# rhofield/rho-tts

Hardware: AMD Instinct MI355X
Metric: audio-sec/wall-sec (RTF) Qwen3-TTS-1.7B batch=32 (higher is better)
Workload: dtype bf16; 1 GPU; Qwen3-TTS-1.7B bf16, batch 32/GPU, 30-s reference clone, 10-word sentences (44 frames each), sampling=top-k 50 T 0.9, seeded synthetic weights; value counts delivered (post-processed) audio; global_batch=32, parallelism=dp1

## Files before the change

### rho_tts_amd/csrc/common.h

```cpp
#pragma once

#include <hip/hip_runtime.h>

#include <cstdarg>
#include <cstdio>
#include <cstring>
#include <atomic>
#include <mutex>
#include <shared_mutex>
#include <string>
#include <vector>

#include "../../include/rho_tts_amd_debug.h"

struct rt_ctx {
    int device = 0;
    hipStream_t own_stream = nullptr;
    hipStream_t stream = nullptr;
    std::mutex mu;
    std::string last_error;
    int n_cu = 0;
    char arch[64] = {0};
    void* d_scratch = nullptr;
    size_t d_scratch_bytes = 0;
// ... 86 lines not shown
    float o;
    o = dpp_lane_f32<0xB1>(v);  v = o > v ? o : v;
    o = dpp_lane_f32<0x4E>(v);  v = o > v ? o : v;
    o = dpp_lane_f32<0x141>(v); v = o > v ? o : v;
    o = dpp_lane_f32<0x140>(v); v = o > v ? o : v;
    const int x = __float_as_int(v);
    const float r0 = __int_as_float(__builtin_amdgcn_readlane(x, 0)), r1 = __int_as_float(__builtin_amdgcn_readlane(x, 16));
    const float r2 = __int_as_float(__builtin_amdgcn_readlane(x, 32)), r3 = __int_as_float(__builtin_amdgcn_readlane(x, 48));
    const float a = r1 > r0 ? r1 : r0, b = r3 > r2 ? r3 : r2;
    return b > a ? b : a;
}
__device__ __forceinline__ unsigned wave_scan_incl_u32(unsigned u) {
    int v = (int)u;
    v += dpp_lane_i32<0x111, true>(v);
    v += dpp_lane_i32<0x112, true>(v);
    v += dpp_lane_i32<0x114, true>(v);
    v += dpp_lane_i32<0x118, true>(v);
    const int t0 = __builtin_amdgcn_readlane(v, 15), t1 = __builtin_amdgcn_readlane(v, 31), t2 = __builtin_amdgcn_readlane(v, 47);
    const int row = (int)(threadIdx.x & 63) >> 4;
    return (unsigned)(v + (row >= 1 ? t0 : 0) + (row >= 2 ? t1 : 0) + (row >= 3 ? t2 : 0));
}
__device__ __forceinline__ float wave_max_f32(float v) {
#pragma unroll
    for (int o = 32; o > 0; o >>= 1) v = fmaxf(v, __shfl_xor(v, o, 64));
    return v;
}
__device__ __forceinline__ int f32_ordered(float f) { const int i = __float_as_int(f); return i >= 0 ? i : i ^ 0x7fffffff; }
__device__ __forceinline__ float ordered_f32(int i) { return __int_as_float(i >= 0 ? i : i ^ 0x7fffffff); }

__host__ __device__ __forceinline__ int64_t tile_off(int m, int k, int K) {
    return ((((int64_t)(m >> 4) * (K >> 5) + (k >> 5)) * 64 + ((((k >> 3) & 3) << 4) | (m & 15))) << 3) + (k & 7);
}

typedef unsigned short bf16_t;
__device__ __forceinline__ float bf16_to_f32(bf16_t v) { return __uint_as_float(((unsigned)v) << 16); }
__device__ __forceinline__ bf16_t f32_to_bf16(float f) {
    const __bf16 b = (__bf16)f;
    return __builtin_bit_cast(bf16_t, b);
}
typedef __attribute__((ext_vector_type(2))) __bf16 rt_bf2_t;
__device__ __forceinline__ unsigned f32x2_to_bf16x2(float lo, float hi) {
    const rt_bf2_t v = {(__bf16)lo, (__bf16)hi};
    return __builtin_bit_cast(unsigned, v);
}

template <int MODE = 0>
__device__ __forceinline__ bool grid_barrier(unsigned* bar, unsigned n_wg, unsigned epoch, unsigned max_spins = 1u << 22) {
    __shared__ int gb_ok;
    if (MODE == 2) __builtin_amdgcn_s_waitcnt(0);
    __syncthreads();
    if (threadIdx.x == 0) {
        if (MODE == 2) __hip_atomic_fetch_add(&bar[0], 1u, __ATOMIC_RELAXED, __HIP_MEMORY_SCOPE_AGENT);
        else __hip_atomic_fetch_add(&bar[0], 1u, __ATOMIC_RELEASE, __HIP_MEMORY_SCOPE_AGENT);
        const unsigned target = epoch * n_wg;
        unsigned spins = 0;
        int good = 1;
        while (__hip_atomic_load(&bar[0], __ATOMIC_RELAXED, __HIP_MEMORY_SCOPE_AGENT) < target) {
            if (++spins > max_spins || __hip_atomic_load(&bar[1], __ATOMIC_RELAXED, __HIP_MEMORY_SCOPE_AGENT) != 0u) {
                __hip_atomic_store(&bar[1], 1u, __ATOMIC_RELAXED, __HIP_MEMORY_SCOPE_AGENT);
                good = 0;
                break;
            }
            __builtin_amdgcn_s_sleep(1);
        }
        gb_ok = good;
        if (MODE == 1) __builtin_amdgcn_fence(__ATOMIC_ACQUIRE, "agent");
// ... 8 lines not shown
```

### rho_tts_amd/csrc/debug.hip

```cpp
#include <algorithm>
#include <vector>

#include "kernels.h"

namespace {
__global__ void k_touch(float* p, int n) {
    const int i = blockIdx.x * blockDim.x + threadIdx.x;
    if (i < n) p[i] = p[i] * 1.0001f + 1.0f;
}
template <int MODE>
__global__ void k_bench_barrier(unsigned* bar, int n, float* buf) {
    const int i = blockIdx.x * blockDim.x + threadIdx.x;
    const int j = (i + blockDim.x) % (gridDim.x * blockDim.x);
    float acc = buf[i];
    for (int e = 1; e <= n; ++e) {
        if (MODE == 2) st_agent(buf + i, acc + 1.0f); else buf[i] = acc + 1.0f;
        if (!grid_barrier<MODE>(bar, gridDim.x, (unsigned)e, 1u << 20)) return;
        acc = MODE == 2 ? ld_agent(buf + j) : buf[j];
        if (acc != (float)e && i == 0) bar[2] = 1u;
    }
    buf[i] = acc;
}
template <int P>
__global__ void k_bench_pair(unsigned* flags, int n, float* buf, unsigned* bar) {
// ... 687 lines not shown
    (void)hipEventDestroy(e0); (void)hipEventDestroy(e1);
    (void)hipFree(wbuf); (void)hipFree(a); (void)hipFree(out);
    return rc;
}

int rt_bench_gemm_col(rt_ctx* ctx, int32_t M, int32_t N, int32_t K, int32_t a_norm, int32_t epi, int32_t n_mats, int32_t iters,
                      double* avg_us, int64_t* stamps8) {
    if (!ctx || !avg_us || M < 1 || M > 128 || N < 64 || K < 16 || K % 16 || n_mats < 1 || iters < 1) return rt_fail(ctx, RT_ERR_INVALID, "rt_bench_gemm_col: bad argument");
    CtxLock g(ctx);
    RT_HIP(ctx, hipSetDevice(ctx->device));
    const size_t pb = packed_bytes(N, K);
    bf16_t* wbuf = nullptr;
    void* a = nullptr;
    float *out = nullptr, *rowsq = nullptr, *rowsq_out = nullptr, *normw = nullptr;
    bf16_t* act = nullptr;
    RT_HIP(ctx, hipMalloc((void**)&wbuf, pb * n_mats));
    const size_t R = M > 64 ? 128 : 64;
    RT_HIP(ctx, hipMalloc(&a, R * K * 4));
    RT_HIP(ctx, hipMalloc((void**)&out, R * N * 4));
    RT_HIP(ctx, hipMalloc((void**)&act, R * N * 2));
    RT_HIP(ctx, hipMalloc((void**)&rowsq, R * 512 * 4));
    RT_HIP(ctx, hipMalloc((void**)&rowsq_out, R * (N / 4 + 4) * 4));
    RT_HIP(ctx, hipMalloc((void**)&normw, (size_t)std::max(K, N) * 4));
    RT_HIP(ctx, hipMemsetAsync(wbuf, 0x3c, pb * n_mats, ctx->stream));
    RT_HIP(ctx, hipMemsetAsync(a, 0x3c, R * K * 4, ctx->stream));
    RT_HIP(ctx, hipMemsetAsync(out, 0, R * N * 4, ctx->stream));
    RT_HIP(ctx, hipMemsetAsync(rowsq, 0x3c, R * 512 * 4, ctx->stream));
    RT_HIP(ctx, hipMemsetAsync(normw, 0x3c, (size_t)std::max(K, N) * 4, ctx->stream));
    PackedW pw;
    pw.N = N; pw.K = K; pw.Np = (N + 31) / 32 * 32; pw.Kp = K; pw.Np16 = (N + 15) / 16 * 16;
    ColArgs c;
    c.nt = (a_norm & 2) ? 0 : 1;
    a_norm &= 1;
    c.A = a; c.post_scale = a_norm; c.rowsq = rowsq; c.rowsq_n = K / 16; c.eps = 1e-6f; c.M = M; c.K = K; c.epi = epi;
    c.next_bf16 = epi == COL_RESID ? act : nullptr; c.next_norm_w = normw;
    c.out = out; c.ldc = epi == COL_SILU ? N / 2 : N; c.split = epi == COL_SILU ? col_split_silu(N, ctx->n_cu) : col_split_for(N, ctx->n_cu);
    c.rowsq_out = rowsq_out; c.rowsq_out_n = N / 16 * c.split; c.out_bf16 = act;
    hipEvent_t e0, e1;
    RT_HIP(ctx, hipEventCreate(&e0));
    RT_HIP(ctx, hipEventCreate(&e1));
    int rc = RT_OK;
    auto launch = [&](const ColArgs& c1) {
        if (c1.M <= 64 || g_col_rows128) return launch_gemm_col(ctx, c1, pw);
        ColArgs lo = c1, hi = c1;
        lo.M = 64; hi.M = c1.M - 64; hi.row_off = 64;
        const int r = launch_gemm_col(ctx, lo, pw);
        return r ? r : launch_gemm_col(ctx, hi, pw);
    };
    for (int i = 0; i < n_mats && !rc; ++i) { pw.data16 = wbuf + (pb / 2) * i; rc = launch(c); }
    RT_HIP(ctx, hipEventRecord(e0, ctx->stream));
    for (int i = 0; i < iters && !rc; ++i) {
        pw.data16 = wbuf + (pb / 2) * (i % n_mats);
        rc = launch(c);
    }
    RT_HIP(ctx, hipEventRecord(e1, ctx->stream));
    RT_HIP(ctx, hipStreamSynchronize(ctx->stream));
    float ms = 0;
    RT_HIP(ctx, hipEventElapsedTime(&ms, e0, e1));
    *avg_us = (double)ms * 1e3 / iters;
    if (stamps8 && !rc) {
        long long* st = nullptr;
        RT_HIP(ctx, hipMalloc((void**)&st, 64));
        RT_HIP(ctx, hipMemsetAsync(st, 0, 64, ctx->stream));
        c.stamps = st;
        pw.data16 = wbuf + (pb / 2) * (iters % n_mats);
        rc = launch_gemm_col(ctx, c, pw);
        RT_HIP(ctx, hipMemcpy(stamps8, st, 64, hipMemcpyDeviceToHost));
        (void)hipFree(st);
    }
    (void)hipEventDestroy(e0); (void)hipEventDestroy(e1);
    (void)hipFree(wbuf); (void)hipFree(a); (void)hipFree(out); (void)hipFree(act); (void)hipFree(rowsq); (void)hipFree(rowsq_out); (void)hipFree(normw);
    return rc;
}

int rt_bench_launch(rt_ctx* ctx, int32_t grid_wgs, int32_t n, int32_t use_graph, int32_t reps, double* us_per_launch) {
    if (!ctx || !us_per_launch || grid_wgs < 1 || n < 1 || reps < 1) return RT_ERR_INVALID;
    CtxLock g(ctx);
    RT_HIP(ctx, hipSetDevice(ctx->device));
    float* buf = nullptr;
    const int elems = grid_wgs * 256;
    RT_HIP(ctx, hipMalloc((void**)&buf, (size_t)elems * 4));
    RT_HIP(ctx, hipMemsetAsync(buf, 0, (size_t)elems * 4, ctx->stream));
    hipEvent_t e0, e1;
    RT_HIP(ctx, hipEventCreate(&e0));
    RT_HIP(ctx, hipEventCreate(&e1));
    hipGraph_t graph = nullptr;
    hipGraphExec_t exec = nullptr;
    if (use_graph) {
        RT_HIP(ctx, hipStreamBeginCapture(ctx->stream, hipStreamCaptureModeThreadLocal));
        for (int i = 0; i < n; ++i) hipLaunchKernelGGL(k_touch, dim3(grid_wgs), dim3(256), 0, ctx->stream, buf, elems);
        RT_HIP(ctx, hipStreamEndCapture(ctx->stream, &graph));
        RT_HIP(ctx, hipGraphInstantiate(&exec, graph, nullptr, nullptr, 0));
        RT_HIP(ctx, hipGraphLaunch(exec, ctx->stream));
        RT_HIP(ctx, hipStreamSynchronize(ctx->stream));
    } else {
        for (int i = 0; i < n; ++i) hipLaunchKernelGGL(k_touch, dim3(grid_wgs), dim3(256), 0, ctx->stream, buf, elems);
        RT_HIP(ctx, hipStreamSynchronize(ctx->stream));
    }
    RT_HIP(ctx, hipEventRecord(e0, ctx->stream));
// ... 166 lines not shown
```

### rho_tts_amd/csrc/gemm_col.hip

```cpp
#include <hip/hip_ext.h>

#include "kernels.h"

namespace {

typedef __attribute__((ext_vector_type(8))) __bf16 bf8_t;
typedef __attribute__((ext_vector_type(8))) short s8_t;
typedef __attribute__((ext_vector_type(16))) float f16_t;
typedef __attribute__((ext_vector_type(4))) float f4_t;
typedef __attribute__((ext_vector_type(4))) int i4_t;

__device__ __forceinline__ f16_t mfma32(s8_t a, s8_t b, f16_t c) {
    return __builtin_amdgcn_mfma_f32_32x32x16_bf16(__builtin_bit_cast(bf8_t, a), __builtin_bit_cast(bf8_t, b), c, 0, 0, 0);
}
__device__ __forceinline__ unsigned pk2(float lo, float hi) { return f32x2_to_bf16x2(lo, hi); }

constexpr int WAVES = 8;

typedef __attribute__((ext_vector_type(4))) float f4acc_t;
__device__ __forceinline__ f4acc_t mfma16(s8_t a, s8_t b, f4acc_t c) {
    return __builtin_amdgcn_mfma_f32_16x16x32_bf16(__builtin_bit_cast(bf8_t, a), __builtin_bit_cast(bf8_t, b), c, 0, 0, 0);
}

constexpr int col_chunk(int epi, int mt, bool x) {
    if (mt == 8) return epi == COL_SILU ? 1 : 2;
    return epi == COL_SILU ? (x ? (mt == 4 ? 2 : 4) : 2) : ((mt == 4 || mt == 1) ? 4 : 8);
}
template <int EPI, int MT, int NPRE, bool X = false, bool NORM = false>
__global__ __launch_bounds__(512, (((EPI == COL_SILU && MT == 2) || MT == 1) && !X) ? 4 : 2) void k_gemm_col(ColArgs g) {
    static_assert(!X || (EPI == COL_SILU && MT >= 2), "the extra half pair exists for gate/up only");
    constexpr int RMT = MT > 4 ? 4 : MT;
    constexpr int ROUNDS = MT / RMT;
    __shared__ float red[WAVES][RMT][4][64];
    __shared__ float sh_inv[16 * MT];
    constexpr int NB = (EPI == COL_SILU) ? (X ? 3 : 2) : 1;
    constexpr int C = col_chunk(EPI, MT, X);
    constexpr int PASSES = (MT + 1) / 2;
    const int tid = threadIdx.x, lane = tid & 63, w = tid >> 6;
    const int r = lane & 15, qd = lane >> 4;
    const int sp_shift = g.split == 4 ? 2 : (g.split == 2 ? 1 : 0);
    const int nt = blockIdx.x >> sp_shift, sub = blockIdx.x & (g.split - 1);
    const int cw_shift = 4 - sp_shift;
    const bool b_mine = (r >> cw_shift) == sub;
    const int kchunk = (g.KT + WAVES - 1) / WAVES;
    const int kt_lo = w * kchunk;
    int kt_hi = kt_lo + kchunk;
    if (kt_hi > g.KT) kt_hi = g.KT;
    const int n_k = kt_hi > kt_lo ? kt_hi - kt_lo : 0;
    const int n_sc = (n_k + C - 1) / C;
    const int n_mt = (g.M + 15) >> 4;

    const s8_t* wp[NB];
    wp[0] = reinterpret_cast<const s8_t*>(g.Wp) + ((int64_t)nt * g.KT + kt_lo) * 64 + lane;
    if (NB >= 2) wp[1] = reinterpret_cast<const s8_t*>(g.Wp) + ((int64_t)(nt + g.up_tile_offset) * g.KT + kt_lo) * 64 + lane;
    const int x_tile = g.x_tile0 + ((int)blockIdx.x >> 1), x_col0 = ((int)blockIdx.x & 1) * 8;
    if (NB == 3) wp[NB - 1] = reinterpret_cast<const s8_t*>(g.Wp) + ((int64_t)(x_tile + (r < 8 ? 0 : g.up_tile_offset)) * g.KT + kt_lo) * 64 + qd * 16 + x_col0 + (r & 7);
    const s8_t* ap[MT];
#pragma unroll
    for (int mt = 0; mt < MT; ++mt) {
        int row = mt * 16 + r;
        if (row >= g.M) row = g.M - 1;
        ap[mt] = reinterpret_cast<const s8_t*>(reinterpret_cast<const bf16_t*>(g.A) + tile_off(g.row_off + row, kt_lo * 32 + qd * 8, g.K));
    }

    struct Chunk {
        s8_t b[NB][C];
        s8_t a[MT][C];
    };
    auto issue = [&](int sc, Chunk& ck) {
#pragma unroll
        for (int u = 0; u < C; ++u) {
            int k = sc * C + u;
            if (k >= n_k) k = n_k - 1;
#pragma unroll
            for (int b = 0; b < NB; ++b) {
                const s8_t zero = {0, 0, 0, 0, 0, 0, 0, 0};
                ck.b[b][u] = !b_mine ? zero : (g.nt ? __builtin_nontemporal_load(wp[b] + (int64_t)k * 64) : wp[b][(int64_t)k * 64]);
            }
#pragma unroll
            for (int mt = 0; mt < MT; ++mt) ck.a[mt][u] = ap[mt][(int64_t)k * 64];
        }
    };

    if (g.stamps && blockIdx.x == 0 && tid == 0) g.stamps[0] = wall_clock64();
    const int e_i = (tid >> 6) & 3, e_l = tid & 63;
    const int n = nt * 16 + (e_l & 15);
    const bool e_mine = ((e_l & 15) >> cw_shift) == sub;
    const bool n_ok = n < g.N && e_mine;
    float rq[PASSES][16];
    constexpr int RQ_MAX = 256;
    if constexpr (NORM) {
#pragma unroll
        for (int ps = 0; ps < PASSES; ++ps) {
            const int row_i = 32 * ps + 4 * w + qd;
            const int row = g.row_off + (row_i < g.M ? row_i : g.M - 1);
            const float* p = g.rowsq + (int64_t)row * g.rowsq_n;
#pragma unroll
            for (int it = 0; it < 16; ++it) {
                const int j = r + 16 * it;
                rq[ps][it] = p[j < g.rowsq_n ? j : g.rowsq_n - 1];
            }
        }
    }
    float xres[PASSES];
    float e_bias = 0.f, e_scale = 1.f, e_nw = 0.f;
    if (n_ok) {
        if (EPI != COL_SILU && g.bias) e_bias = g.bias[n];
        if (EPI == COL_RESID && g.scale) e_scale = g.scale[n];
        if (EPI == COL_RESID && g.next_bf16) e_nw = g.next_norm_w[n];
    }
#pragma unroll
    for (int ps = 0; ps < PASSES; ++ps) {
        const int e_row = (2 * ps + (tid >> 8)) * 16 + (e_l >> 4) * 4 + e_i;
        xres[ps] = 0.f;
        if (EPI == COL_RESID && e_row < g.M && n_ok) xres[ps] = g.out[tile_off(g.row_off + e_row, n, (int)g.ldc)];
    }
    __builtin_amdgcn_sched_barrier(0);
    Chunk c0, c1;
    if (NPRE >= 1 || n_sc > 0) issue(0, c0);
    if (NPRE >= 2 || (NPRE == 0 && n_sc > 1)) issue(1, c1);
    __builtin_amdgcn_sched_barrier(0);
    if constexpr (NORM) {
#pragma unroll
        for (int ps = 0; ps < PASSES; ++ps) {
            const int row_i = 32 * ps + 4 * w + qd;
            float s = 0.f;
#pragma unroll
            for (int it = 0; it < 16; ++it) s += (r + 16 * it < g.rowsq_n) ? rq[ps][it] : 0.f;
            if (g.rowsq_n > RQ_MAX) {
                const int row = g.row_off + (row_i < g.M ? row_i : g.M - 1);
                const float* p = g.rowsq + (int64_t)row * g.rowsq_n;
                for (int j = RQ_MAX + r; j < g.rowsq_n; j += 16) s += p[j];
            }
            s = group_sum_f32<16>(s);
            if (r == 0 && row_i < 16 * MT) sh_inv[row_i] = rsqrtf(s / (float)g.K + g.eps);
        }
    }
    if (g.stamps && blockIdx.x == 0 && tid == 0) g.stamps[1] = wall_clock64();

    f4acc_t acc[NB][MT];
#pragma unroll
    for (int b = 0; b < NB; ++b)
#pragma unroll
        for (int mt = 0; mt < MT; ++mt)
#pragma unroll
            for (int i = 0; i < 4; ++i) acc[b][mt][i] = 0.f;

    auto consume = [&](int sc, Chunk& ck) {
#pragma unroll
        for (int u = 0; u < C; ++u) {
            if (sc * C + u < n_k) {
#pragma unroll
                for (int b = 0; b < NB; ++b)
#pragma unroll
                    for (int mt = 0; mt < MT; ++mt)
                        if (mt == 0 || mt < n_mt) acc[b][mt] = mfma16(ck.a[mt][u], ck.b[b][u], acc[b][mt]);
            }
        }
    };
    for (int sc = 0; sc < n_sc; sc += 2) {
        consume(sc, c0);
        if (g.stamps && sc == 0 && blockIdx.x == 0 && tid == 0) g.stamps[2] = wall_clock64();
// ... 22 lines not shown
                const int smt = 2 * pp + (tid >> 8);
                if (smt < RMT) {
#pragma unroll
                    for (int ww = 0; ww < WAVES; ++ww) s += red[ww][smt < RMT ? smt : 0][e_i][e_l];
                }
                val[b][rd * (RMT / 2) + pp] = s;
            }
        }
    }
    if (g.stamps && blockIdx.x == 0 && tid == 0) g.stamps[4] = wall_clock64();
#pragma unroll
    for (int ps = 0; ps < PASSES; ++ps) {
        const int e_row = (2 * ps + (tid >> 8)) * 16 + (e_l >> 4) * 4 + e_i;
        const bool ok = e_row < g.M && n_ok;
        const float inv = (NORM && e_row < 16 * MT) ? sh_inv[e_row] : 1.f;
        float v = val[0][ps] * inv;
        if (EPI == COL_STORE) {
            if (ok) {
                v += e_bias;
                g.out[(int64_t)(g.row_off + e_row) * g.ldc + n] = v;
            }
        } else if (EPI == COL_RESID) {
            float xn = 0.f;
            if (ok) {
                v += e_bias;
                v *= e_scale;
                xn = xres[ps] + v;
                const int64_t o = tile_off(g.row_off + e_row, n, (int)g.ldc);
                g.out[o] = xn;
                if (g.next_bf16) g.next_bf16[o] = f32_to_bf16(e_nw * xn);
            }
            float sq = xn * xn;
            sq = group_sum_f32<16>(sq);
            if ((e_l & 15) == 0 && e_row < g.M) g.rowsq_out[(int64_t)(g.row_off + e_row) * g.rowsq_out_n + blockIdx.x] = sq;
        } else {
            if (ok) {
                const float u = val[1][ps] * inv;
                g.out_bf16[tile_off(g.row_off + e_row, n, (int)g.ldc)] = f32_to_bf16(v / (1.f + __expf(-v)) * u);
            }
            if (X) {
                const float gx = val[NB - 1][ps] * inv;
                const float ux = __shfl_down(gx, 8, 16);
                const int nx = x_tile * 16 + x_col0 + (e_l & 7);
                if (e_row < g.M && (e_l & 15) < 8 && nx < g.N) g.out_bf16[tile_off(g.row_off + e_row, nx, (int)g.ldc)] = f32_to_bf16(gx / (1.f + __expf(-gx)) * ux);
            }
        }
    }
    if (g.stamps && blockIdx.x == 0 && tid == 0) g.stamps[5] = wall_clock64();
}

template <int EPI, int MT, int NPRE, bool X, bool NORM>
void launch_one(rt_ctx* ctx, const ColArgs& g, dim3 grid, hipEvent_t e0, hipEvent_t e1) {
    if (!e0 && !e1) hipLaunchKernelGGL((k_gemm_col<EPI, MT, NPRE, X, NORM>), grid, dim3(512), 0, ctx->stream, g);
    else hipExtLaunchKernelGGL((k_gemm_col<EPI, MT, NPRE, X, NORM>), grid, dim3(512), 0, ctx->stream, e0, e1, 0, g);
}

template <int EPI, int MT, bool X, bool NORM>
void launch_npre2(rt_ctx* ctx, const ColArgs& g, dim3 grid, hipEvent_t e0, hipEvent_t e1) {
    constexpr int C = col_chunk(EPI, MT, X);
    const int kchunk = (g.KT + WAVES - 1) / WAVES;
    const bool all_waves_busy = g.KT >= WAVES && (WAVES - 1) * kchunk < g.KT;
    const int n_sc = (kchunk + C - 1) / C;
    if (!all_waves_busy) launch_one<EPI, MT, 0, X, NORM>(ctx, g, grid, e0, e1);
    else if (n_sc >= 2) launch_one<EPI, MT, 2, X, NORM>(ctx, g, grid, e0, e1);
    else launch_one<EPI, MT, 1, X, NORM>(ctx, g, grid, e0, e1);
}

template <int EPI, int MT, bool X = false>
void launch_npre(rt_ctx* ctx, const ColArgs& g, dim3 grid, hipEvent_t e0, hipEvent_t e1) {
    if (g.post_scale) {
        if constexpr (EPI != COL_RESID) launch_npre2<EPI, MT, X, true>(ctx, g, grid, e0, e1);
    } else {
        launch_npre2<EPI, MT, X, false>(ctx, g, grid, e0, e1);
    }
}

int dispatch_epi(rt_ctx* ctx, const ColArgs& g, dim3 grid, hipEvent_t e0, hipEvent_t e1) {
    const bool wide = g.M > 32, narrow = g.M <= 16 && g_col_rows16;
    if (g.M > 64) {
        switch (g.epi) {
            case COL_STORE: launch_npre<COL_STORE, 8>(ctx, g, grid, e0, e1); break;
            case COL_RESID: launch_npre<COL_RESID, 8>(ctx, g, grid, e0, e1); break;
            case COL_SILU:
                if (g.x_tile0 > 0) launch_npre<COL_SILU, 8, true>(ctx, g, grid, e0, e1);
                else launch_npre<COL_SILU, 8>(ctx, g, grid, e0, e1);
                break;
            default: return rt_fail(ctx, RT_ERR_INVALID, "gemm_col: bad epilogue %d", g.epi);
        }
        RT_HIP(ctx, hipGetLastError());
        return RT_OK;
    }
    switch (g.epi) {
        case COL_STORE: wide ? launch_npre<COL_STORE, 4>(ctx, g, grid, e0, e1) : narrow ? launch_npre<COL_STORE, 1>(ctx, g, grid, e0, e1) : launch_npre<COL_STORE, 2>(ctx, g, grid, e0, e1); break;
        case COL_RESID: wide ? launch_npre<COL_RESID, 4>(ctx, g, grid, e0, e1) : narrow ? launch_npre<COL_RESID, 1>(ctx, g, grid, e0, e1) : launch_npre<COL_RESID, 2>(ctx, g, grid, e0, e1); break;
        case COL_SILU:
            if (g.x_tile0 > 0) wide ? launch_npre<COL_SILU, 4, true>(ctx, g, grid, e0, e1) : launch_npre<COL_SILU, 2, true>(ctx, g, grid, e0, e1);
            else wide ? launch_npre<COL_SILU, 4>(ctx, g, grid, e0, e1) : narrow ? launch_npre<COL_SILU, 1>(ctx, g, grid, e0, e1) : launch_npre<COL_SILU, 2>(ctx, g, grid, e0, e1);
            break;
        default: return rt_fail(ctx, RT_ERR_INVALID, "gemm_col: bad epilogue %d", g.epi);
    }
    RT_HIP(ctx, hipGetLastError());
    return RT_OK;
}

}

int col_split_silu(int N, int n_cu) {
    (void)N; (void)n_cu;
    return (g_col_split == 2 || g_col_split == 4) ? g_col_split.load() : 1;
}

int col_split_for(int N, int n_cu) {
    if (g_col_split == 1 || g_col_split == 2 || g_col_split == 4) return g_col_split;
    const int tiles = (N + 15) / 16;
    if (g_col_split4 && tiles * 4 <= n_cu) return 4;
    if (tiles * 2 <= n_cu) return 2;
    return 1;
}

int launch_gemm_col(rt_ctx* ctx, const ColArgs& a, const PackedW& w, hipEvent_t ev_start, hipEvent_t ev_stop) {
    if (a.M < 1 || a.M > 128) return rt_fail(ctx, RT_ERR_INVALID, "gemm_col: M=%d outside 1..128 (callers split larger row blocks)", a.M);
    if (w.K != a.K || w.K % 32) return rt_fail(ctx, RT_ERR_INVALID, "gemm_col: K mismatch (%d vs %d) or not a multiple of 32", w.K, a.K);
    if (!w.data16) return rt_fail(ctx, RT_ERR_STATE, "gemm_col: weight has no 16-column decode copy");
    ColArgs g = a;
    g.Wp = w.data16;
    g.NT = w.Np16 / 16;
    g.KT = w.K / 32;
    if (g.split != 1 && g.split != 2 && g.split != 4) return rt_fail(ctx, RT_ERR_INVALID, "gemm_col: split %d (1, 2 or 4)", g.split);
    int tiles = g.NT;
    if (g.epi == COL_SILU) {
        if (w.N % 32) return rt_fail(ctx, RT_ERR_INVALID, "gemm_col: gate/up width %d not a multiple of 32", w.N);
        tiles = g.NT / 2;
        g.up_tile_offset = g.NT / 2;
        g.N = w.N / 2;
        g.x_tile0 = 0;
        const int wg = tiles / 3 * 2;
        const bool narrow = g.M <= 16 && g_col_rows16;
        if (g_col_silu_x && g.split == 1 && !narrow && tiles % 3 == 0 && tiles > ctx->n_cu && wg <= ctx->n_cu && (w.N / 2) % 16 == 0) {
            g.x_tile0 = wg;
            tiles = wg;
        }
    } else {
        g.N = w.N;
    }
    if (g.epi == COL_RESID && (!g.rowsq_out || g.rowsq_out_n < g.NT * g.split)) return rt_fail(ctx, RT_ERR_INVALID, "gemm_col: rowsq_out too small");
    if (g.post_scale && (!g.rowsq || g.rowsq_n < 1)) return rt_fail(ctx, RT_ERR_INVALID, "gemm_col: row scaling without partials");
    if (g.post_scale && g.epi == COL_RESID) return rt_fail(ctx, RT_ERR_UNSUPPORTED, "gemm_col: the residual epilogue has no row-scaled instantiation");
    if (g.next_bf16 && !g.next_norm_w) return rt_fail(ctx, RT_ERR_INVALID, "gemm_col: next operand without its norm weight");
    return dispatch_epi(ctx, g, dim3(tiles * g.split), ev_start, ev_stop);
}
```

### rho_tts_amd/csrc/kernels.h

```cpp
#pragma once
#include "common.h"
#include "knobs.h"

struct PackedW {
    const bf16_t* data = nullptr;
    int N = 0, K = 0;
    int Np = 0, Kp = 0;
    size_t bytes() const { return (size_t)Np * Kp * 2; }
    const bf16_t* data16 = nullptr;
    int Np16 = 0;
};

struct GemmA {
    const void* ptr = nullptr;
    const void* ptr_lo = nullptr;
    int is_f32 = 0;
    int split = 0;
    int64_t M = 0;
    int Cin = 0;
    int taps = 1;
    int tap_stride = 1;
    int tap_offset = 0;
    int rows_out = 0;
    int rows_in = 0;
// ... 33 lines not shown
bool gemm_mid_shape_ok(int N, int K);
int launch_gemm_mid(rt_ctx* ctx, const bf16_t* A, int M, const PackedW& w, float* out, int64_t ldc);
int launch_gemm_skinny(rt_ctx* ctx, const bf16_t* d_a, int M, const PackedW& w, float* d_out, int64_t ldc, int split_k,
                       hipEvent_t ev_start = nullptr, hipEvent_t ev_stop = nullptr, int64_t slab_stride = 0);
int skinny_pick_split(int M, int N, int K, int n_cu);
int col_split_for(int N, int n_cu);
int col_split_silu(int N, int n_cu);

enum { COL_STORE = 0, COL_RESID = 1, COL_SILU = 2 };
struct ColArgs {
    int row_off = 0;
    const void* A = nullptr;
    int nt = 1;
    int post_scale = 0;
    const float* rowsq = nullptr;
    int rowsq_n = 0;
    float eps = 0.f;
    int M = 0, K = 0;
    int epi = COL_STORE;
    int split = 1;
    float* out = nullptr;
    bf16_t* next_bf16 = nullptr;
    const float* next_norm_w = nullptr;
    int64_t ldc = 0;
    const float* bias = nullptr;
    const float* scale = nullptr;
    float* rowsq_out = nullptr;
    int rowsq_out_n = 0;
    bf16_t* out_bf16 = nullptr;
    long long* stamps = nullptr;
    const bf16_t* Wp = nullptr;
    int NT = 0, KT = 0, N = 0, up_tile_offset = 0;
    int x_tile0 = 0;
};
int launch_gemm_col(rt_ctx* ctx, const ColArgs& a, const PackedW& w, hipEvent_t ev_start = nullptr, hipEvent_t ev_stop = nullptr);
struct RowsqGather {
    const float* table = nullptr;
    const int32_t* idx = nullptr;
    int idx_stride = 1, first = 0;
    const int32_t* frame_ptr = nullptr;
    int64_t idx_frame_stride = 0;
};
int launch_rowsq(rt_ctx* ctx, const float* x, int M, int H, float* rowsq, int rowsq_n, float* x_tiled = nullptr,
                 bf16_t* a_tiled = nullptr, const float* norm_w = nullptr, const int32_t* src_rows = nullptr,
                 const int32_t* dst_rows = nullptr, const RowsqGather* gather = nullptr);

struct GatherSrc;
int launch_embed_rowsq(rt_ctx* ctx, const GatherSrc* d_srcs, int n_src, const float* f32_table, const int32_t* d_idx, int idx_stride,
                       const int32_t* frame_ptr, int64_t idx_frame_stride, int M, int H, const float* add_vec, float* rowsq, int rowsq_n,
                       float* x_tiled, bf16_t* a_tiled, const float* norm_w, int32_t* frame_inc = nullptr, unsigned* arrive = nullptr,
                       const float* qkv_table = nullptr, float* qkv_out = nullptr, int qkv_n = 0);

int launch_norm_tiled_rows(rt_ctx* ctx, const float* x_tiled, const float* rowsq, int rowsq_n, const float* w, float eps, int M, int H,
                           float* out);

int launch_add_rmsnorm(rt_ctx* ctx, float* x, int M, int H, const float* slabs, int n_slabs, const float* slab_bias,
                       const float* scale, const float* w, float eps, bf16_t* out_bf16, float* out_f32);
int launch_silu_mul(rt_ctx* ctx, const float* slabs, int n_slabs, int M, int I, bf16_t* out, float* out_f32 = nullptr);
int launch_reduce_slabs(rt_ctx* ctx, const float* slabs, int n_slabs, int64_t M, int N, const float* bias, int act,
                        float* out_f32, bf16_t* out_bf16);

struct KvCache {
    bf16_t* k = nullptr;
    bf16_t* v = nullptr;
    int layers = 0, slots = 0, kv_heads = 0, max_pos = 0, head_dim = 0;
    bf16_t* k_lo = nullptr;
    bf16_t* v_lo = nullptr;
// ... 103 lines not shown
```

### rho_tts_amd/csrc/knobs.h

```cpp
#pragma once
#include "common.h"

#define RT_KNOBS(X) \
    X(0, g_skinny_variant, 0, 0, 2, "legacy skinny GEMM: 0 k_gemm_skinny, 1 k_gemm_skinny2<.,4>, 2 k_gemm_skinny2<.,8>") \
    X(100, g_decode_col, 1, 0, 1, "0 legacy 9-launch split-K decode, 1 column-owner GEMM + fused attention (5 launches per layer)") \
    X(200, g_use_graph, 1, 0, 1, "0 eager decode frames, 1 replayed from captured hipGraphs") \
    X(300, g_pred_nt, 0, 0, 1, "predictor weights: 0 cacheable loads (Infinity-Cache resident across its 15 passes), 1 non-temporal") \
    X(400, g_decode_lanes, 1, 1, 8, "decode lanes: groups of items decoding concurrently on their own streams (rt_generate)") \
    X(500, g_col_split, 0, 0, 4, "sub-tile split of narrow decode GEMMs: 0 automatic (col_split_for), 1 / 2 / 4 forced") \
    X(600, g_tile96, 1, 0, 1, "1: 128x96 workgroup tiles for N = 96 / 192 (codec decoder), 0: always 128x128") \
    X(700, g_col_rows64, 1, 0, 1, "1: one 64-row decode GEMM launch for the predictor's two-position pass, 0: two 32-row launches") \
    X(800, g_fuse_sample_embed, 1, 0, 1, "1: sampler + next-input embedding in one launch (predictor groups), 0: separate k_embed_rowsq") \
    X(900, g_prefill_fill, 3, 0, 99, "workgroups per CU a prefill GEMM's split-K aims for") \
    X(1000, g_xcd_order, 1, 0, 1, "1: tiled GEMMs run a row tile's column tiles back to back on one XCD") \
    X(1100, g_final_conv, 1, 0, 1, "the codec decoder's last conv: 1 its own LDS-window kernel, 0 a one-column GEMM") \
    X(1200, g_conv_win, 1, 0, 1, "1: k>1 convs on operand planes keep their input window in LDS (k_conv_win), 0: per-tap kernel") \
    X(1300, g_sync_parts, 0, 0, 1, "1: rt_generate waits for the stream after every frame part (bounds the dispatches in flight; profiling aid)") \
    X(1400, g_eos_check_every, 8, 1, 99, "frames between two host looks at the device-side end-of-sequence flags (1 = every frame)") \
    X(1500, g_attn_mfma, 0, 0, 2, "the talker's shared-prefix decode attention: 0 vector unit, 1 / 2 matrix cores with four rows / one row per workgroup (attention_mfma.hip); 1 measured " \
        "16.6 us per launch against 13.3 us for the vector-unit kernel at batch 32 / 460 prefix rows, so off") \
    X(1600, g_col_split4, 0, 0, 1, "1: the automatic split may go to quarter tiles (N <= 1024 on 256 CUs); measured 1.4 ms/step slower than half tiles") \
    X(1700, g_handover_every, 4, 1, 99, "queued items (n_items > rows): frames between two looks at the flags + row hand-overs.  Measured on the 1.7B model, 512 / 64 ragged texts on 32 " \
        "rows: 2 -> 487 / 445, 3 -> 489 / 445, 4 -> 491 / 447, 6 -> 485 / 445, 8 -> 477 / 428, 12 -> 475 / 434 audio-s/s (a hand-over costs ~1.4 ms, a waiting row 0.13 ms per frame)") \
    X(1800, g_conv_tall, 1, 0, 2, "k>1 convs of the 96- / 192-channel stages: 0 128-row tiles, 1 256-row tiles for long inputs, 2 always") \
    X(1900, g_prefill_mid, 1, 0, 3, "prompt prefills of 65..1024 rows: 0 split-K tiled kernel, 1 k_gemm_mid (no split-K slabs), 2 / 3 force its 64 / 128 tiles") \
    X(2000, g_col_max_rows, 64, 1, 64, "batches of up to 64 rows decode on the column-owner path while they have at most this many rows (65..128 rows always do, and only while this stands at 64).  Above 32 the talker's GEMMs take 64 rows per launch and the predictor's " \
        "two-position first pass runs as two 64-row launches: 715 audio-s/s at batch 64 against 510 at batch 32 (1.7B, bench.py --batch 64) - every weight byte serves twice the rows for " \
        "~1.4x the launch time") \
    X(2100, g_fuse_conv, 1, 0, 1, "1: a 96-channel k>1 conv and the 1x1 conv behind its activation run as one launch (launch_conv_pair); 0 switches the 192-channel pairs off as well") \
    X(2200, g_prefill_attn_mfma, 1, 0, 1, "prompt attention behind a shared voice prefix: 0 vector unit, 1 matrix cores") \
    X(2300, g_col_rows16, 0, 0, 1, "1: decode GEMM launches of <= 16 rows take the 128-VGPR MT = 1 instantiation (two workgroups per CU: decode lanes)") \
    X(2400, g_col_silu_x, 1, 0, 1, "1: gate/up GEMMs whose pairs are 1.5x the CUs run as one round of 1.5-pair workgroups, 0: one pair per workgroup (1.5 rounds)") \
    X(2600, g_conv_unroll, 1, 0, 1, "1: k = 7 convs run the tap-unrolled instantiation of k_conv_win, 0: the generic tap loop") \
    X(2700, g_frame_inc_fold, 0, 0, 1, "1: frame += 1 by the last workgroup of the frame's talker-input launch, 0: k_frame_inc (the fold measured 1-1.8 ms per step SLOWER)") \
    X(2800, g_pair_attn, 1, 0, 1, "1: two-position decode passes append both positions inside the fused attention launch, 0: k_qkv_post + k_attention") \
    X(2900, g_c2w_lean, 1, 0, 1, "1: rt_code2wav drops the third unit's unread residual-stream store and the waveform copy (the last conv writes the caller's buffer)") \
    X(3000, g_fuse_conv192, 1, 0, 1, "1: the 192-channel conv pairs fuse as well, weight fragments staged through LDS") \
    X(3100, g_pred_qkv_table, 1, 0, 1, "predictor passes 2..G-1: 1 layer 0's q/k/v row of the drawn code is copied from the table rt_model_finalize builds (by the launch " \
        "that embeds the code), 0 the layer-0 qkv GEMM launch runs (same bits either way)") \
    X(3200, g_col_rows128, 1, 0, 1, "generations on 65..128 rows: 1 one 128-row decode GEMM launch per weight matrix (k_gemm_col MT = 8: the weights are streamed once), " \
        "0 two 64-row launches (same bits either way).  Measured (1.7B, profiles/r18_rows128.txt): bench.py --corpus 512 --batch 128 1014 audio-s/s with 1 against 887 with 0 (five alternating pairs; 824 on 64 rows); " \
        "per launch at 128 rows qkv 13.7 / 16.3 us, o 12.0 / 14.2, gate/up 20.9 / 27.4, down 27.3 / 29.7 (one launch / two)") \
    X(3300, g_stt_gather_ranged, 1, 0, 1, "speech-to-text under a prompt policy, the gather between beam steps: 1 the ranged form (generated positions only; the prefix " \
        "sits in both caches), 0 the uniform form over [0, longest prefix of the group + step) (same bits either way; profiles/r20_stt_prompt.txt)")

#define RT_KNOB_ARG(X) \
    X(0, g_skinny_waves_per_cu, 4, 1, 0x7fffffff, "legacy skinny GEMM: split-K is chosen so that about this many waves per CU stream weights")

#define RT_KNOB_EXTERN(base, name, def, lo, hi, doc) extern rt_knob name;
RT_KNOBS(RT_KNOB_EXTERN)
RT_KNOB_ARG(RT_KNOB_EXTERN)
#undef RT_KNOB_EXTERN
extern std::atomic<int> g_tune_epoch;
```

### rho_tts_amd/csrc/rowops.hip

```cpp
#include "kernels.h"

namespace {

typedef __attribute__((ext_vector_type(4))) float f4_t;

__device__ __forceinline__ float block_sum_f32(float v, float* sh) {
    v = wave_sum_f32(v);
    const int w = threadIdx.x >> 6, nw = (blockDim.x + 63) >> 6;
    __syncthreads();
    if ((threadIdx.x & 63) == 0) sh[w] = v;
    __syncthreads();
    float t = 0.f;
    for (int i = 0; i < nw; ++i) t += sh[i];
    return t;
}

__global__ __launch_bounds__(256) void k_add_rmsnorm(float* __restrict__ x, int H, const float* __restrict__ slabs, int n_slabs,
                                                     int64_t slab_stride, const float* __restrict__ slab_bias,
                                                     const float* __restrict__ scale, const float* __restrict__ w, float eps,
                                                     bf16_t* __restrict__ out_bf16, float* __restrict__ out_f32) {
    __shared__ float sh[4];
    constexpr int MAXV = 8;
    const int64_t row = blockIdx.x;
    const int nv = H >> 2;
// ... 203 lines not shown
                for (int e = 0; e < 4; ++e) {
                    v[2 * e] += __uint_as_float(wds[e] << 16);
                    v[2 * e + 1] += __uint_as_float(wds[e] & 0xffff0000u);
                }
            }
        }
#pragma unroll
        for (int e = 0; e < 8; ++e) ss += v[e] * v[e];
        const int64_t o = tile_off(row, c, H);
        *reinterpret_cast<f4_t*>(x_tiled + o) = f4_t{v[0], v[1], v[2], v[3]};
        *reinterpret_cast<f4_t*>(x_tiled + o + 4) = f4_t{v[4], v[5], v[6], v[7]};
        const f4_t w0 = *reinterpret_cast<const f4_t*>(norm_w + c), w1 = *reinterpret_cast<const f4_t*>(norm_w + c + 4);
        uint4 pk;
        pk.x = f32x2_to_bf16x2(w0[0] * v[0], w0[1] * v[1]);
        pk.y = f32x2_to_bf16x2(w0[2] * v[2], w0[3] * v[3]);
        pk.z = f32x2_to_bf16x2(w1[0] * v[4], w1[1] * v[5]);
        pk.w = f32x2_to_bf16x2(w1[2] * v[6], w1[3] * v[7]);
        *reinterpret_cast<uint4*>(a_tiled + o) = pk;
    }
    if (qkv_table) {
        f4_t* qdst = reinterpret_cast<f4_t*>(qkv_out + (int64_t)row * qkv_n);
#pragma unroll
        for (int u = 0; u < QU; ++u) {
            const int i = tid + u * 256;
            if (i < n4) qdst[i] = qv[u];
        }
        for (int i = tid + QU * 256; i < n4; i += 256) qdst[i] = qsrc[i];
    }
    const float tot = block_sum_f32(ss, sh);
    for (int j = tid; j < rowsq_n; j += 256) rowsq[(int64_t)row * rowsq_n + j] = j == 0 ? tot : 0.f;
}

__global__ __launch_bounds__(256) void k_norm_tiled_rows(const float* __restrict__ x_tiled, const float* __restrict__ rowsq, int rowsq_n,
                                                         const float* __restrict__ w, float eps, int H, float* __restrict__ out) {
    __shared__ float sh[4];
    const int row = blockIdx.x;
    float s = 0.f;
    for (int j = threadIdx.x; j < rowsq_n; j += 256) s += rowsq[(int64_t)row * rowsq_n + j];
    const float inv = rsqrtf(block_sum_f32(s, sh) / (float)H + eps);
    for (int c = threadIdx.x * 4; c < H; c += 1024) {
        const f4_t v = *reinterpret_cast<const f4_t*>(x_tiled + tile_off(row, c, H));
        const f4_t wv = *reinterpret_cast<const f4_t*>(w + c);
        *reinterpret_cast<f4_t*>(out + (int64_t)row * H + c) = f4_t{wv[0] * (v[0] * inv), wv[1] * (v[1] * inv), wv[2] * (v[2] * inv), wv[3] * (v[3] * inv)};
    }
}

__global__ void k_silu_mul(const float* __restrict__ slabs, int n_slabs, int64_t slab_stride, int I, bf16_t* __restrict__ out,
                           int64_t total4, float* __restrict__ out_f32) {
    const int I4 = I >> 2;
    for (int64_t idx = (int64_t)blockIdx.x * blockDim.x + threadIdx.x; idx < total4; idx += (int64_t)gridDim.x * blockDim.x) {
        const int64_t m = idx / I4;
        const int i = (int)(idx - m * I4);
        f4_t g = {0.f, 0.f, 0.f, 0.f}, u = {0.f, 0.f, 0.f, 0.f};
        const f4_t* p = reinterpret_cast<const f4_t*>(slabs + m * 2 * I);
        const int64_t st4 = slab_stride >> 2;
#pragma unroll 8
        for (int s = 0; s < n_slabs; ++s) {
            g += p[s * st4 + i];
            u += p[s * st4 + I4 + i];
        }
        float r[4];
#pragma unroll
        for (int j = 0; j < 4; ++j) r[j] = g[j] / (1.f + __expf(-g[j])) * u[j];
        if (out_f32) { reinterpret_cast<f4_t*>(out_f32)[idx] = f4_t{r[0], r[1], r[2], r[3]}; continue; }
        uint2 pk;
        pk.x = (unsigned)f32_to_bf16(r[0]) | ((unsigned)f32_to_bf16(r[1]) << 16);
        pk.y = (unsigned)f32_to_bf16(r[2]) | ((unsigned)f32_to_bf16(r[3]) << 16);
        reinterpret_cast<uint2*>(out)[idx] = pk;
    }
}

// ... 223 lines not shown

int launch_rowsq(rt_ctx* ctx, const float* x, int M, int H, float* rowsq, int rowsq_n, float* x_tiled, bf16_t* a_tiled,
                 const float* norm_w, const int32_t* src_rows, const int32_t* dst_rows, const RowsqGather* gather) {
    if (M <= 0) return RT_OK;
    const RowsqGather gt = gather ? *gather : RowsqGather{};
    if (gt.table && (src_rows || dst_rows || gt.first < 0 || gt.first > M || !gt.idx))
        return rt_fail(ctx, RT_ERR_INVALID, "rowsq: gathered rows take no row maps (first %d of %d rows)", gt.first, M);
    hipLaunchKernelGGL(k_rowsq, dim3(M), dim3(256), 0, ctx->stream, x, H, rowsq, rowsq_n, x_tiled, a_tiled, norm_w, src_rows, dst_rows, gt);
    RT_HIP(ctx, hipGetLastError());
    return RT_OK;
}

int launch_embed_rowsq(rt_ctx* ctx, const GatherSrc* d_srcs, int n_src, const float* f32_table, const int32_t* d_idx, int idx_stride,
                       const int32_t* frame_ptr, int64_t idx_frame_stride, int M, int H, const float* add_vec, float* rowsq, int rowsq_n,
                       float* x_tiled, bf16_t* a_tiled, const float* norm_w, int32_t* frame_inc, unsigned* arrive, const float* qkv_table,
                       float* qkv_out, int qkv_n) {
    if (M <= 0) return RT_OK;
    if (n_src > 16 || H % 8 || !x_tiled || !a_tiled || !norm_w || !rowsq || rowsq_n < 1 || (n_src > 0 && !d_srcs))
        return rt_fail(ctx, RT_ERR_INVALID, "embed_rowsq: n_src %d (<= 16), H %d (multiple of 8) or a missing buffer", n_src, H);
    if (frame_inc && (f32_table || !arrive || frame_inc != frame_ptr))
        return rt_fail(ctx, RT_ERR_INVALID, "embed_rowsq: the frame counter is advanced by launches over bf16 sources only, with an arrival counter");
    if (qkv_table && (!qkv_out || qkv_n < 4 || qkv_n % 4 || frame_inc || (f32_table ? n_src != 0 : n_src != 1)))
        return rt_fail(ctx, RT_ERR_INVALID, "embed_rowsq: the q/k/v table takes one code per row, an output and a row width that is a multiple of 4");
    hipLaunchKernelGGL(k_embed_rowsq, dim3(M), dim3(256), 0, ctx->stream, d_srcs, n_src, f32_table, d_idx, idx_stride, frame_ptr,
                       idx_frame_stride, H, add_vec, rowsq, rowsq_n, x_tiled, a_tiled, norm_w, frame_inc, arrive, qkv_table, qkv_out, qkv_n);
    RT_HIP(ctx, hipGetLastError());
    return RT_OK;
}

int launch_norm_tiled_rows(rt_ctx* ctx, const float* x_tiled, const float* rowsq, int rowsq_n, const float* w, float eps, int M, int H,
                           float* out) {
    if (M <= 0) return RT_OK;
    if (H % 8) return rt_fail(ctx, RT_ERR_INVALID, "norm_tiled_rows: H %d not a multiple of 8", H);
    hipLaunchKernelGGL(k_norm_tiled_rows, dim3(M), dim3(256), 0, ctx->stream, x_tiled, rowsq, rowsq_n, w, eps, H, out);
    RT_HIP(ctx, hipGetLastError());
    return RT_OK;
}

int launch_silu_mul(rt_ctx* ctx, const float* slabs, int n_slabs, int M, int I, bf16_t* out, float* out_f32) {
    const int64_t total = (int64_t)M * I / 4;
    if (total <= 0) return RT_OK;
    if (I % 4) return rt_fail(ctx, RT_ERR_UNSUPPORTED, "silu_mul: intermediate size %d not a multiple of 4", I);
    hipLaunchKernelGGL(k_silu_mul, dim3(grid_for(total, 64)), dim3(64), 0, ctx->stream, slabs, n_slabs, (int64_t)M * 2 * I, I, out, total, out_f32);
    RT_HIP(ctx, hipGetLastError());
    return RT_OK;
}

int launch_reduce_slabs(rt_ctx* ctx, const float* slabs, int n_slabs, int64_t M, int N, const float* bias, int act, float* out_f32,
                        bf16_t* out_bf16) {
    const int64_t total = M * N;
    if (total <= 0) return RT_OK;
    hipLaunchKernelGGL(k_reduce_slabs, dim3(grid_for(total)), dim3(256), 0, ctx->stream, slabs, n_slabs, total, N, bias, act, out_f32,
                       out_bf16, total);
    RT_HIP(ctx, hipGetLastError());
    return RT_OK;
}

int launch_qkv_post(rt_ctx* ctx, const float* slabs, int n_slabs, int M, int heads, int kv_heads, int head_dim, const float* q_norm_w,
                    const float* k_norm_w, float eps, const float* rope_cos, const float* rope_sin, const int32_t* row_slot,
                    const int32_t* row_pos, int pos_add, float* q_out, const KvCache& kv, int layer, const int32_t* frame_ptr) {
    if (M <= 0) return RT_OK;
    if (head_dim > 128 || (head_dim & 1)) return rt_fail(ctx, RT_ERR_UNSUPPORTED, "head_dim %d unsupported (even, <= 128)", head_dim);
    const int width = (heads + 2 * kv_heads) * head_dim;
    hipLaunchKernelGGL(k_qkv_post, dim3(M, heads + 2 * kv_heads), dim3(64), 0, ctx->stream, slabs, n_slabs, (int64_t)M * width, heads,
                       kv_heads, head_dim, q_norm_w, k_norm_w, eps, rope_cos, rope_sin, row_slot, row_pos, pos_add, q_out,
                       kv.k + layer * kv.layer_stride(), kv.v + layer * kv.layer_stride(), kv.max_pos, frame_ptr,
                       kv.k_lo ? kv.k_lo + layer * kv.layer_stride() : nullptr, kv.v_lo ? kv.v_lo + layer * kv.layer_stride() : nullptr);
// ... 61 lines not shown
```

Before: 576.5 audio-s/s.

## Permute rowsq partials for wide prologue loads and fit GEMM chunk lengths

```diff
diff --git a/rho_tts_amd/csrc/common.h b/rho_tts_amd/csrc/common.h
--- a/rho_tts_amd/csrc/common.h
+++ b/rho_tts_amd/csrc/common.h
@@ -142,6 +142,10 @@
     return ((((int64_t)(m >> 4) * (K >> 5) + (k >> 5)) * 64 + ((((k >> 3) & 3) << 4) | (m & 15))) << 3) + (k & 7);
 }
 
+__host__ __device__ __forceinline__ int rowsq_slot(int j, int n) {
+    return (n & 63) ? j : (64 * (j >> 6) + 4 * (j & 15) + ((j >> 4) & 3));
+}
+
 typedef unsigned short bf16_t;
 __device__ __forceinline__ float bf16_to_f32(bf16_t v) { return __uint_as_float(((unsigned)v) << 16); }
 __device__ __forceinline__ bf16_t f32_to_bf16(float f) {
diff --git a/rho_tts_amd/csrc/debug.hip b/rho_tts_amd/csrc/debug.hip
--- a/rho_tts_amd/csrc/debug.hip
+++ b/rho_tts_amd/csrc/debug.hip
@@ -743,7 +743,7 @@
     ColArgs c;
     c.nt = (a_norm & 2) ? 0 : 1;
     a_norm &= 1;
-    c.A = a; c.post_scale = a_norm; c.rowsq = rowsq; c.rowsq_n = K / 16; c.eps = 1e-6f; c.M = M; c.K = K; c.epi = epi;
+    c.A = a; c.post_scale = a_norm; c.rowsq = rowsq; c.rowsq_n = K / 16 * col_split_for(K, ctx->n_cu); c.eps = 1e-6f; c.M = M; c.K = K; c.epi = epi;
     c.next_bf16 = epi == COL_RESID ? act : nullptr; c.next_norm_w = normw;
     c.out = out; c.ldc = epi == COL_SILU ? N / 2 : N; c.split = epi == COL_SILU ? col_split_silu(N, ctx->n_cu) : col_split_for(N, ctx->n_cu);
     c.rowsq_out = rowsq_out; c.rowsq_out_n = N / 16 * c.split; c.out_bf16 = act;
@@ -776,6 +776,7 @@
         c.stamps = st;
         pw.data16 = wbuf + (pb / 2) * (iters % n_mats);
         rc = launch_gemm_col(ctx, c, pw);
+        RT_HIP(ctx, hipStreamSynchronize(ctx->stream));
         RT_HIP(ctx, hipMemcpy(stamps8, st, 64, hipMemcpyDeviceToHost));
         (void)hipFree(st);
     }
diff --git a/rho_tts_amd/csrc/gemm_col.hip b/rho_tts_amd/csrc/gemm_col.hip
--- a/rho_tts_amd/csrc/gemm_col.hip
+++ b/rho_tts_amd/csrc/gemm_col.hip
@@ -26,7 +26,7 @@
     if (mt == 8) return epi == COL_SILU ? 1 : 2;
     return epi == COL_SILU ? (x ? (mt == 4 ? 2 : 4) : 2) : ((mt == 4 || mt == 1) ? 4 : 8);
 }
-template <int EPI, int MT, int NPRE, bool X = false, bool NORM = false>
+template <int EPI, int MT, int NPRE, bool X = false, bool NORM = false, int WQ = 0, int CF = 0>
 __global__ __launch_bounds__(512, (((EPI == COL_SILU && MT == 2) || MT == 1) && !X) ? 4 : 2) void k_gemm_col(ColArgs g) {
     static_assert(!X || (EPI == COL_SILU && MT >= 2), "the extra half pair exists for gate/up only");
     constexpr int RMT = MT > 4 ? 4 : MT;
@@ -34,7 +34,9 @@
     __shared__ float red[WAVES][RMT][4][64];
     __shared__ float sh_inv[16 * MT];
     constexpr int NB = (EPI == COL_SILU) ? (X ? 3 : 2) : 1;
-    constexpr int C = col_chunk(EPI, MT, X);
+    static_assert(WQ == 0 || NORM, "wide requests exist for the row-scale partials only");
+    static_assert(CF == 0 || (EPI != COL_SILU && MT == 2), "fitted chunks exist for STORE / RESID launches of up to 32 rows only");
+    constexpr int C = CF ? CF : col_chunk(EPI, MT, X);
     constexpr int PASSES = (MT + 1) / 2;
     const int tid = threadIdx.x, lane = tid & 63, w = tid >> 6;
     const int r = lane & 15, qd = lane >> 4;
@@ -87,9 +89,20 @@
     const int n = nt * 16 + (e_l & 15);
     const bool e_mine = ((e_l & 15) >> cw_shift) == sub;
     const bool n_ok = n < g.N && e_mine;
-    float rq[PASSES][16];
+    float rq[PASSES][WQ ? 1 : 16];
+    f4_t rq4[PASSES][WQ ? WQ : 1];
     constexpr int RQ_MAX = 256;
-    if constexpr (NORM) {
+    if constexpr (NORM && WQ > 0) {
+        const int q_last = (g.rowsq_n >> 6) - 1;
+#pragma unroll
+        for (int ps = 0; ps < PASSES; ++ps) {
+            const int row_i = 32 * ps + 4 * w + qd;
+            const int row = g.row_off + (row_i < g.M ? row_i : g.M - 1);
+            const f4_t* p = reinterpret_cast<const f4_t*>(g.rowsq + (int64_t)row * g.rowsq_n) + r;
+#pragma unroll
+            for (int q = 0; q < WQ; ++q) rq4[ps][q] = p[16 * (q < q_last ? q : q_last)];
+        }
+    } else if constexpr (NORM) {
 #pragma unroll
         for (int ps = 0; ps < PASSES; ++ps) {
             const int row_i = 32 * ps + 4 * w + qd;
@@ -125,9 +138,14 @@
         for (int ps = 0; ps < PASSES; ++ps) {
             const int row_i = 32 * ps + 4 * w + qd;
             float s = 0.f;
-#pragma unroll
-            for (int it = 0; it < 16; ++it) s += (r + 16 * it < g.rowsq_n) ? rq[ps][it] : 0.f;
-            if (g.rowsq_n > RQ_MAX) {
+            if constexpr (WQ > 0) {
+#pragma unroll
+                for (int it = 0; it < 4 * WQ; ++it) s += (r + 16 * it < g.rowsq_n) ? rq4[ps][it >> 2][it & 3] : 0.f;
+            } else {
+#pragma unroll
+                for (int it = 0; it < 16; ++it) s += (r + 16 * it < g.rowsq_n) ? rq[ps][it] : 0.f;
+            }
+            if (WQ == 0 && g.rowsq_n > RQ_MAX) {
                 const int row = g.row_off + (row_i < g.M ? row_i : g.M - 1);
                 const float* p = g.rowsq + (int64_t)row * g.rowsq_n;
                 for (int j = RQ_MAX + r; j < g.rowsq_n; j += 16) s += p[j];
@@ -216,7 +234,7 @@
             }
             float sq = xn * xn;
             sq = group_sum_f32<16>(sq);
-            if ((e_l & 15) == 0 && e_row < g.M) g.rowsq_out[(int64_t)(g.row_off + e_row) * g.rowsq_out_n + blockIdx.x] = sq;
+            if ((e_l & 15) == 0 && e_row < g.M) g.rowsq_out[(int64_t)(g.row_off + e_row) * g.rowsq_out_n + (g.rowsq_perm ? rowsq_slot((int)blockIdx.x, g.rowsq_out_n) : (int)blockIdx.x)] = sq;
         } else {
             if (ok) {
                 const float u = val[1][ps] * inv;
@@ -233,29 +251,43 @@
     if (g.stamps && blockIdx.x == 0 && tid == 0) g.stamps[5] = wall_clock64();
 }
 
-template <int EPI, int MT, int NPRE, bool X, bool NORM>
+template <int EPI, int MT, int NPRE, bool X, bool NORM, int WQ, int CF>
 void launch_one(rt_ctx* ctx, const ColArgs& g, dim3 grid, hipEvent_t e0, hipEvent_t e1) {
-    if (!e0 && !e1) hipLaunchKernelGGL((k_gemm_col<EPI, MT, NPRE, X, NORM>), grid, dim3(512), 0, ctx->stream, g);
-    else hipExtLaunchKernelGGL((k_gemm_col<EPI, MT, NPRE, X, NORM>), grid, dim3(512), 0, ctx->stream, e0, e1, 0, g);
-}
-
-template <int EPI, int MT, bool X, bool NORM>
+    if (!e0 && !e1) hipLaunchKernelGGL((k_gemm_col<EPI, MT, NPRE, X, NORM, WQ, CF>), grid, dim3(512), 0, ctx->stream, g);
+    else hipExtLaunchKernelGGL((k_gemm_col<EPI, MT, NPRE, X, NORM, WQ, CF>), grid, dim3(512), 0, ctx->stream, e0, e1, 0, g);
+}
+
+template <int EPI, int MT, bool X, bool NORM, int WQ, int CF>
 void launch_npre2(rt_ctx* ctx, const ColArgs& g, dim3 grid, hipEvent_t e0, hipEvent_t e1) {
-    constexpr int C = col_chunk(EPI, MT, X);
+    constexpr int C = CF ? CF : col_chunk(EPI, MT, X);
     const int kchunk = (g.KT + WAVES - 1) / WAVES;
     const bool all_waves_busy = g.KT >= WAVES && (WAVES - 1) * kchunk < g.KT;
     const int n_sc = (kchunk + C - 1) / C;
-    if (!all_waves_busy) launch_one<EPI, MT, 0, X, NORM>(ctx, g, grid, e0, e1);
-    else if (n_sc >= 2) launch_one<EPI, MT, 2, X, NORM>(ctx, g, grid, e0, e1);
-    else launch_one<EPI, MT, 1, X, NORM>(ctx, g, grid, e0, e1);
+    if (!all_waves_busy) launch_one<EPI, MT, 0, X, NORM, WQ, CF>(ctx, g, grid, e0, e1);
+    else if (n_sc >= 2) launch_one<EPI, MT, 2, X, NORM, WQ, CF>(ctx, g, grid, e0, e1);
+    else launch_one<EPI, MT, 1, X, NORM, WQ, CF>(ctx, g, grid, e0, e1);
+}
+
+template <int EPI, int MT, bool X, bool NORM, int WQ>
+void launch_chunk(rt_ctx* ctx, const ColArgs& g, dim3 grid, hipEvent_t e0, hipEvent_t e1) {
+    if constexpr (EPI != COL_SILU && MT == 2) {
+        const int kchunk = (g.KT + WAVES - 1) / WAVES;
+        if (g_col_chunk_fit && kchunk <= 4) return launch_npre2<EPI, MT, X, NORM, WQ, 4>(ctx, g, grid, e0, e1);
+        if (g_col_chunk_fit && kchunk > 8 && kchunk <= 12) return launch_npre2<EPI, MT, X, NORM, WQ, 6>(ctx, g, grid, e0, e1);
+    }
+    launch_npre2<EPI, MT, X, NORM, WQ, 0>(ctx, g, grid, e0, e1);
 }
 
 template <int EPI, int MT, bool X = false>
 void launch_npre(rt_ctx* ctx, const ColArgs& g, dim3 grid, hipEvent_t e0, hipEvent_t e1) {
     if (g.post_scale) {
-        if constexpr (EPI != COL_RESID) launch_npre2<EPI, MT, X, true>(ctx, g, grid, e0, e1);
+        if constexpr (EPI != COL_RESID) {
+            if (g.rowsq_wide == 2) launch_chunk<EPI, MT, X, true, 2>(ctx, g, grid, e0, e1);
+            else if (g.rowsq_wide == 4) launch_chunk<EPI, MT, X, true, 4>(ctx, g, grid, e0, e1);
+            else launch_chunk<EPI, MT, X, true, 0>(ctx, g, grid, e0, e1);
+        }
     } else {
-        launch_npre2<EPI, MT, X, false>(ctx, g, grid, e0, e1);
+        launch_chunk<EPI, MT, X, false, 0>(ctx, g, grid, e0, e1);
     }
 }
 
@@ -301,6 +333,8 @@
     if (tiles * 2 <= n_cu) return 2;
     return 1;
 }
+
+bool rowsq_permuted(int n) { return g_rowsq_wide && n % 64 == 0 && n >= 64 && n <= 256; }
 
 int launch_gemm_col(rt_ctx* ctx, const ColArgs& a, const PackedW& w, hipEvent_t ev_start, hipEvent_t ev_stop) {
     if (a.M < 1 || a.M > 128) return rt_fail(ctx, RT_ERR_INVALID, "gemm_col: M=%d outside 1..128 (callers split larger row blocks)", a.M);
@@ -331,5 +365,9 @@
     if (g.post_scale && (!g.rowsq || g.rowsq_n < 1)) return rt_fail(ctx, RT_ERR_INVALID, "gemm_col: row scaling without partials");
     if (g.post_scale && g.epi == COL_RESID) return rt_fail(ctx, RT_ERR_UNSUPPORTED, "gemm_col: the residual epilogue has no row-scaled instantiation");
     if (g.next_bf16 && !g.next_norm_w) return rt_fail(ctx, RT_ERR_INVALID, "gemm_col: next operand without its norm weight");
+    g.rowsq_perm = (g.epi == COL_RESID && rowsq_permuted(g.rowsq_out_n)) ? 1 : 0;
+    g.rowsq_wide = (g.post_scale && rowsq_permuted(g.rowsq_n)) ? (g.rowsq_n <= 128 ? 2 : 4) : 0;
+    if (g.rowsq_wide && (reinterpret_cast<uintptr_t>(g.rowsq) & 15))
+        return rt_fail(ctx, RT_ERR_INVALID, "gemm_col: rowsq rows read in 16-byte pieces must be 16-byte aligned");
     return dispatch_epi(ctx, g, dim3(tiles * g.split), ev_start, ev_stop);
 }
diff --git a/rho_tts_amd/csrc/kernels.h b/rho_tts_amd/csrc/kernels.h
--- a/rho_tts_amd/csrc/kernels.h
+++ b/rho_tts_amd/csrc/kernels.h
@@ -89,7 +89,10 @@
     const bf16_t* Wp = nullptr;
     int NT = 0, KT = 0, N = 0, up_tile_offset = 0;
     int x_tile0 = 0;
-};
+    int rowsq_perm = 0;
+    int rowsq_wide = 0;
+};
+bool rowsq_permuted(int n);
 int launch_gemm_col(rt_ctx* ctx, const ColArgs& a, const PackedW& w, hipEvent_t ev_start = nullptr, hipEvent_t ev_stop = nullptr);
 struct RowsqGather {
     const float* table = nullptr;
diff --git a/rho_tts_amd/csrc/knobs.h b/rho_tts_amd/csrc/knobs.h
--- a/rho_tts_amd/csrc/knobs.h
+++ b/rho_tts_amd/csrc/knobs.h
@@ -42,7 +42,12 @@
         "0 two 64-row launches (same bits either way).  Measured (1.7B, profiles/r18_rows128.txt): bench.py --corpus 512 --batch 128 1014 audio-s/s with 1 against 887 with 0 (five alternating pairs; 824 on 64 rows); " \
         "per launch at 128 rows qkv 13.7 / 16.3 us, o 12.0 / 14.2, gate/up 20.9 / 27.4, down 27.3 / 29.7 (one launch / two)") \
     X(3300, g_stt_gather_ranged, 1, 0, 1, "speech-to-text under a prompt policy, the gather between beam steps: 1 the ranged form (generated positions only; the prefix " \
-        "sits in both caches), 0 the uniform form over [0, longest prefix of the group + step) (same bits either way; profiles/r20_stt_prompt.txt)")
+        "sits in both caches), 0 the uniform form over [0, longest prefix of the group + step) (same bits either way; profiles/r20_stt_prompt.txt)") \
+    X(3400, g_rowsq_wide, 1, 0, 1, "RMSNorm sum-of-squares partials of the decode GEMMs, rows of n partials with n % 64 == 0 and n <= 256: 1 stored permuted (rowsq_slot) " \
+        "and fetched by the row-scale prologue in 2 / 4 16-byte requests per lane, 0 stored plainly and fetched in 16 dword requests (same bits either way; " \
+        "profiles/r21_gemm_col_prologue.txt)") \
+    X(3500, g_col_chunk_fit, 1, 0, 1, "STORE / RESID decode GEMM launches of up to 32 rows: 1 the chunk length follows the wave's run of k-tiles (one chunk of 4 for K <= 1024, " \
+        "two of 6 for K = 3072: no clamped re-loads of the run's last tile), 0 chunks of 8 (same bits either way; profiles/r21_gemm_col_prologue.txt)")
 
 #define RT_KNOB_ARG(X) \
     X(0, g_skinny_waves_per_cu, 4, 1, 0x7fffffff, "legacy skinny GEMM: split-K is chosen so that about this many waves per CU stream weights")
diff --git a/rho_tts_amd/csrc/rowops.hip b/rho_tts_amd/csrc/rowops.hip
--- a/rho_tts_amd/csrc/rowops.hip
+++ b/rho_tts_amd/csrc/rowops.hip
@@ -259,11 +259,11 @@
 }
 
 __global__ __launch_bounds__(256) void k_norm_tiled_rows(const float* __restrict__ x_tiled, const float* __restrict__ rowsq, int rowsq_n,
-                                                         const float* __restrict__ w, float eps, int H, float* __restrict__ out) {
+                                                         const float* __restrict__ w, float eps, int H, float* __restrict__ out, int perm) {
     __shared__ float sh[4];
     const int row = blockIdx.x;
     float s = 0.f;
-    for (int j = threadIdx.x; j < rowsq_n; j += 256) s += rowsq[(int64_t)row * rowsq_n + j];
+    for (int j = threadIdx.x; j < rowsq_n; j += 256) s += rowsq[(int64_t)row * rowsq_n + (perm ? rowsq_slot(j, rowsq_n) : j)];
     const float inv = rsqrtf(block_sum_f32(s, sh) / (float)H + eps);
     for (int c = threadIdx.x * 4; c < H; c += 1024) {
         const f4_t v = *reinterpret_cast<const f4_t*>(x_tiled + tile_off(row, c, H));
@@ -553,7 +553,8 @@
                            float* out) {
     if (M <= 0) return RT_OK;
     if (H % 8) return rt_fail(ctx, RT_ERR_INVALID, "norm_tiled_rows: H %d not a multiple of 8", H);
-    hipLaunchKernelGGL(k_norm_tiled_rows, dim3(M), dim3(256), 0, ctx->stream, x_tiled, rowsq, rowsq_n, w, eps, H, out);
+    hipLaunchKernelGGL(k_norm_tiled_rows, dim3(M), dim3(256), 0, ctx->stream, x_tiled, rowsq, rowsq_n, w, eps, H, out,
+                       rowsq_permuted(rowsq_n) ? 1 : 0);
     RT_HIP(ctx, hipGetLastError());
     return RT_OK;
 }
```

Result: faster. 594.2 audio-s/s (median of 6 runs) (+3.1%).
